# JerryX1110/Robust-Video-Object-Segmentation

Hardware: AMD Instinct MI355X
Metric: frames/sec, AOC-Net matching + calibration hot path (480p, 3 objects) (higher is better)
Workload: dtype f32; 1 GPU; cfg2: 121x213 stride-4 maps (480p), O=4 (3 objects + background), K=16 proxies, C=100, 60-frame clips, MEM_EVERY=5 (pool R=1..12), 20 Lloyd iterations, local windows 2..12, 10 IA gates + 4 conditioning blocks; sequences_per_gpu=2, proxy_mode=reference

## Files before the change

robust-video-object-segmentation_amd/csrc/labels_kmeans.hip:

```cpp
#include "aoc_common.h"
#include <stdlib.h>
#include <algorithm>

namespace {

constexpr int LP_BLOCK = 256;

__global__ __launch_bounds__(LP_BLOCK) void label_flags_kernel(const float *__restrict__ labels, int n, int n_obj,
                                                                uint32_t *__restrict__ right_bits,
                                                                uint32_t *__restrict__ wrong_bits,
                                                                int32_t *__restrict__ block_counts, int n_blocks) {
    __shared__ int32_t wave_cnt[LP_BLOCK / 64][AOC_MAX_OBJECTS + 1];
    const int row = blockIdx.x * LP_BLOCK + threadIdx.x;
    uint32_t right = 0, wrong = 0;
    if (row < n) {
        const float *l = labels + (size_t)row * n_obj;
        float sum = 0.0f;
        for (int o = 0; o < n_obj; ++o) {
            float v = l[o];
            sum += v;
            if (v > 0.9f) right |= 1u << o;
            if (v < 0.1f) wrong |= 1u << o;
        }
        if (sum > 0.9f) right |= AOC_ROW_KEPT_BIT;
// ... 285 lines not shown
        }
        float v[KU_G][NF];
#pragma unroll
        for (int u = 0; u < KU_G; ++u) {
            const float *base = pool + (size_t)r[u] * C;
#pragma unroll
            for (int f = 0; f < NF; ++f) {
                int t = lane + 64 * f;
                v[u][f] = (t < C) ? base[t] : 0.0f;
            }
        }
#pragma unroll
        for (int u = 0; u < KU_G; ++u) {
            const bool on = u < nmem;
#pragma unroll
            for (int f = 0; f < NF; ++f) acc[f] = acc[f] + (on ? v[u][f] : 0.0f);
        }
        qhead += nmem;
    };

    for (int base = 0; base < len; base += 64) {
        const int p = base + lane;
        const bool valid = p < len;
        const int lab = valid ? labels[beg + p] : -1;
        int row;
        if (MODE == 0) row = valid ? rows[beg + p] : 0;
        else row = valid ? rows[p] : 0;
        const bool mine = lab == j;
        const unsigned long long m = __ballot(mine);
        const int nm = __popcll(m);
        if (nm == 0) continue;
        if (mine) ring[(qtail + __popcll(m & lt)) & (KU_RING - 1)] = row;
        qtail += nm;
        cnt += nm;
        while (qtail - qhead >= KU_G) drain(KU_G);
    }
    while (qtail - qhead > 0) drain(min(KU_G, qtail - qhead));

    if (MODE == 0) {
        if (lane == 0) cluster_counts[s * kmax + j] = cnt;
        if (cnt == 0) return;
        const float fc = (float)cnt;
        float *dst = centroids + ((size_t)s * kmax + j) * C;
#pragma unroll
        for (int f = 0; f < NF; ++f) {
            int t = lane + 64 * f;
            float q = acc[f] / fc;
            if (t < C) { dst[t] = q; stage[t] = q; }
        }
        __syncthreads();
        if (lane == 0) cnorm[s * kmax + j] = sqnorm_seq(stage, C);
    } else {
        const float *csrc = centroids + ((size_t)s * kmax + j) * C;
        float *p0 = proxies + (((size_t)s * 2 + 0) * kmax + j) * C;
        float *p1 = proxies + (((size_t)s * 2 + 1) * kmax + j) * C;
        float n0 = 0.0f, n1 = 0.0f;
#pragma unroll
        for (int f = 0; f < NF; ++f) {
            int t = lane + 64 * f;
            if (t < C) {
                float c = csrc[t];
                p0[t] = c;
                n0 += c * c;
                float a = (cnt > 0) ? acc[f] / (float)cnt : 0.0f;
                p1[t] = a;
                n1 += a * a;
            }
        }
        n0 = aoc_wave_sum(n0);
        n1 = aoc_wave_sum(n1);
        if (lane == 0) {
            proxy_sqnorm[((size_t)s * 2 + 0) * kmax + j] = n0;
            proxy_sqnorm[((size_t)s * 2 + 1) * kmax + j] = (cnt > 0) ? n1 : INFINITY;
        }
    }
}

typedef uint32_t u32x4 __attribute__((ext_vector_type(4)));
typedef uint32_t u32x2 __attribute__((ext_vector_type(2)));
constexpr uint32_t KU_INVALID_OFF = 0xFFFFFF00u;

#ifdef AOC_KS_STATS
__device__ unsigned long long aoc_ks_stats[8];
#define KS_STAT(i, n) do { if (threadIdx.x == 0) atomicAdd(&aoc_ks_stats[i], (unsigned long long)(n)); } while (0)
#else
#define KS_STAT(i, n) do { } while (0)
#endif
#ifdef AOC_KS_STATS
#define KS_CLK() ((long long)__builtin_readcyclecounter())
#else
#define KS_CLK() 0ll
#endif
constexpr int KS_T = 8;

__device__ __forceinline__ int ks_wave_sum(int v) {
    v += __builtin_amdgcn_update_dpp(0, v, 0x111, 0xf, 0xf, true);
    v += __builtin_amdgcn_update_dpp(0, v, 0x112, 0xf, 0xf, true);
    v += __builtin_amdgcn_update_dpp(0, v, 0x114, 0xf, 0xf, true);
    v += __builtin_amdgcn_update_dpp(0, v, 0x118, 0xf, 0xf, true);
    return __builtin_amdgcn_readlane(v, 15) + __builtin_amdgcn_readlane(v, 31) + __builtin_amdgcn_readlane(v, 47) +
           __builtin_amdgcn_readlane(v, 63);
}

__device__ __forceinline__ void ks_fold_block(float x, float inv_u, int lane, int &accr, int &par, unsigned long long &badmask) {
    const float y = x * inv_u;
    const float rn = rintf(y);
    int r = (int)rn;
    badmask |= __ballot(!(__float_as_uint(y) < 0x4B800000u));
    const unsigned long long ties = __ballot(fabsf(rn - y) == 0.5f);
    if (ties) {
        const int fl = (int)floorf(y);
        if ((ties >> lane) & 1ull) r = fl;
        const unsigned long long odd = __ballot((r & 1) != 0);
        int base_par = par, from = 0;
        unsigned long long tm = ties;
        while (tm) {
            const int t = __builtin_ctzll(tm);
            tm &= tm - 1;
            const unsigned long long below_t = (t == 0) ? 0ull : (~0ull >> (64 - t));
            const unsigned long long below_from = (from == 0) ? 0ull : (~0ull >> (64 - from));
            const int pb = base_par ^ (__popcll(odd & below_t & ~below_from) & 1);
            const int bump = pb ^ (int)((odd >> t) & 1ull);
            if (lane == t) r += bump;
            base_par = 0;
            from = t + 1;
        }
        const unsigned long long rest = (from >= 64) ? 0ull : (~0ull << from);
        par = base_par ^ (__popcll(odd & rest) & 1);
    } else {
        par ^= __popcll(__ballot((r & 1) != 0)) & 1;
    }
    accr += r;
}

struct KsBinade {
    float u, inv_u;
    int n_in;
    bool ok;
};
__device__ __forceinline__ KsBinade ks_binade(float s) {
    KsBinade b;
    const uint32_t bits = __float_as_uint(s);
    const int e = (int)((bits >> 23) & 0xff) - 127;
    b.ok = (s > 0.0f) && e >= -100 && e <= 100;
    const int ee = b.ok ? e : 0;
    b.u = __uint_as_float((uint32_t)(ee - 23 + 127) << 23);
    b.inv_u = __uint_as_float((uint32_t)(23 - ee + 127) << 23);
    b.n_in = (int)(s * b.inv_u);
    return b;
}

__device__ __forceinline__ float ks_serial_block(float s, float x, int from = 0) {
    if (__ballot(x != 0.0f) == 0ull) return s;
    for (int kk = from; kk < 64; ++kk) s = s + __uint_as_float(__builtin_amdgcn_readlane(__float_as_uint(x), kk));
    return s;
}

__device__ __forceinline__ int ks_wave_scan(int v) {
    v += __builtin_amdgcn_update_dpp(0, v, 0x111, 0xf, 0xf, true);
    v += __builtin_amdgcn_update_dpp(0, v, 0x112, 0xf, 0xf, true);
    v += __builtin_amdgcn_update_dpp(0, v, 0x114, 0xf, 0xf, true);
    v += __builtin_amdgcn_update_dpp(0, v, 0x118, 0xf, 0xf, true);
    v += __builtin_amdgcn_update_dpp(0, v, 0x142, 0xa, 0xf, false);
    v += __builtin_amdgcn_update_dpp(0, v, 0x143, 0xc, 0xf, false);
    return v;
}

__device__ __forceinline__ float ks_block_exact(float s, float x, int lane) {
    int from = 0;
#pragma unroll 1
    for (int round = 0; round < 4; ++round) {
        const KsBinade bb = ks_binade(s);
        if (!bb.ok) break;
        int r = 0, pr = bb.n_in & 1;
        unsigned long long bd = 0ull;
        ks_fold_block((lane >= from) ? x : 0.0f, bb.inv_u, lane, r, pr, bd);
        if (bd != 0ull) break;
        const int pre = ks_wave_scan(r);
        const int total = __builtin_amdgcn_readlane(pre, 63);
        if ((long long)bb.n_in + total <= 0xFFFFFF) return (float)(bb.n_in + total) * bb.u;
        const unsigned long long over = __ballot((long long)bb.n_in + pre > 0xFFFFFF);
        const int mstar = __builtin_ctzll(over);
        const int before = (mstar == 0) ? 0 : __builtin_amdgcn_readlane(pre, mstar - 1);
        const float s_before = (float)(bb.n_in + before) * bb.u;
        s = s_before + __uint_as_float(__builtin_amdgcn_readlane(__float_as_uint(x), mstar));
        from = mstar + 1;
        if (from >= 64) return s;
    }
    return ks_serial_block(s, x, from);
}

template <int C4MAX>
__global__ __launch_bounds__(256) void km_assign_rank_kernel(const float *__restrict__ pool, int C, const int32_t *__restrict__ rows,
                                                              const int32_t *__restrict__ seg_off, const int32_t *__restrict__ seg_k,
                                                              const float *__restrict__ centroids, int kmax, int32_t *__restrict__ labels,
                                                              uint16_t *__restrict__ rank16, int32_t *__restrict__ hist, int nb_max,
                                                              float *__restrict__ rownorm, int first_iter) {
    extern __shared__ __attribute__((aligned(16))) float lds[];
    const int s = blockIdx.y;
    const int k = seg_k[s];
    if (k <= 0) return;
    const int beg = seg_off[s];
    const int len = seg_off[s + 1] - beg;
    if ((int)(blockIdx.x * 256) >= len) return;
    const int c4 = C >> 2;
    float *lc = lds;
    float *lcn = lds + (size_t)k * C;
    int32_t *wcnt = reinterpret_cast<int32_t *>(lcn + kmax);
    const float *csrc = centroids + (size_t)s * kmax * C;
    for (int i = threadIdx.x; i < k * C; i += 256) lc[i] = csrc[i];
    __syncthreads();
    if ((int)threadIdx.x < k) lcn[threadIdx.x] = sqnorm_seq(lc + (size_t)threadIdx.x * C, C);
    __syncthreads();
    const int p = blockIdx.x * 256 + threadIdx.x;
    const bool valid = p < len;
    int best = -1;
    if (valid) {
        const float4 *xr = reinterpret_cast<const float4 *>(pool + (size_t)rows[beg + p] * C);
        float4 x[C4MAX];
#pragma unroll
        for (int t = 0; t < C4MAX; ++t) x[t] = (t < c4) ? xr[t] : make_float4(0.f, 0.f, 0.f, 0.f);
        float xs;
        if (first_iter) {
            xs = 0.0f;
#pragma unroll
            for (int t = 0; t < C4MAX; ++t) {
                if (t < c4) {
                    float p0 = x[t].x * x[t].x; xs = xs + p0;
                    float p1 = x[t].y * x[t].y; xs = xs + p1;
                    float p2 = x[t].z * x[t].z; xs = xs + p2;
                    float p3 = x[t].w * x[t].w; xs = xs + p3;
                }
            }
            rownorm[beg + p] = xs;
        } else {
            xs = rownorm[beg + p];
        }
        float low = INFINITY;
        best = 0;
        for (int j = 0; j < k; ++j) {
            const float4 *cj = reinterpret_cast<const float4 *>(lc + (size_t)j * C);
            float acc = 0.0f;
#pragma unroll
            for (int t = 0; t < C4MAX; ++t) {
                if (t < c4) {
                    float4 c = cj[t];
                    acc = __builtin_fmaf(x[t].x, c.x, acc);
                    acc = __builtin_fmaf(x[t].y, c.y, acc);
                    acc = __builtin_fmaf(x[t].z, c.z, acc);
                    acc = __builtin_fmaf(x[t].w, c.w, acc);
                }
            }
            float m = -2.0f * acc;
            float dist = (m + xs) + lcn[j];
            if (dist < low) { low = dist; best = j; }
        }
        labels[beg + p] = best;
    }
    const int lane = aoc_lane(), wave = threadIdx.x >> 6;
    const unsigned long long lt = (lane == 0) ? 0ull : (~0ull >> (64 - lane));
    int rank = 0;
    for (int kk = 0; kk < k; ++kk) {
        const unsigned long long m = __ballot(best == kk);
        if (best == kk) rank = __popcll(m & lt);
        if (lane == 0) wcnt[wave * kmax + kk] = __popcll(m);
    }
    __syncthreads();
    if (valid) {
        int woff = 0;
        for (int w = 0; w < wave; ++w) woff += wcnt[w * kmax + best];
        rank16[beg + p] = (uint16_t)(woff + rank);
    }
    if ((int)threadIdx.x < k)
        hist[((size_t)s * nb_max + blockIdx.x) * kmax + threadIdx.x] =
            wcnt[threadIdx.x] + wcnt[kmax + threadIdx.x] + wcnt[2 * kmax + threadIdx.x] + wcnt[3 * kmax + threadIdx.x];
}

__global__ __launch_bounds__(256) void km_rownorm_kernel(const float *__restrict__ pool, int C, const int32_t *__restrict__ rows,
                                                          const int32_t *__restrict__ seg_off, int n_seg_limit, float *__restrict__ rownorm) {
    const int total = seg_off[n_seg_limit];
    const int i = blockIdx.x * 256 + threadIdx.x;
    if (i >= total) return;
    const float4 *xr = reinterpret_cast<const float4 *>(pool + (size_t)rows[i] * C);
    const int c4 = C >> 2;
    float xs = 0.0f;
    for (int t0 = 0; t0 < c4; t0 += 5) {
        float4 v[5];
#pragma unroll
        for (int u = 0; u < 5; ++u) v[u] = xr[min(t0 + u, c4 - 1)];
#pragma unroll
        for (int u = 0; u < 5; ++u) {
            if (t0 + u < c4) {
                float p0 = v[u].x * v[u].x; xs = xs + p0;
                float p1 = v[u].y * v[u].y; xs = xs + p1;
                float p2 = v[u].z * v[u].z; xs = xs + p2;
                float p3 = v[u].w * v[u].w; xs = xs + p3;
            }
        }
    }
    rownorm[i] = xs;
}

constexpr int KA_TPF4 = 1;
template <int TMAX, int KT>
__global__ __launch_bounds__(256, KT == 1 ? 3 : 2) void km_assign_mfma_kernel(const float *__restrict__ pool, int C, const int32_t *__restrict__ rows,
                                                              const int32_t *__restrict__ seg_off, const int32_t *__restrict__ seg_k, int n_seg,
                                                              const float *__restrict__ centroids, int kmax, int32_t *__restrict__ labels,
                                                              uint16_t *__restrict__ rank16, int32_t *__restrict__ hist, int nb_max,
                                                              const float *__restrict__ rownorm) {
    extern __shared__ __attribute__((aligned(16))) float lds[];
    constexpr int TP = (TMAX + 3) / 4 * 4;
    constexpr int RS = 4 * TP + 4;
    constexpr int NB4 = TP / 4;
    constexpr int PIECES = (16 * TMAX + 63) / 64;
    constexpr int c4 = TMAX;
    const int lane = aoc_lane(), wave = threadIdx.x >> 6;
    const int j = lane & 15, g = lane >> 4;

    float *cimg = lds;
    float *lcn = cimg + (size_t)KT * 16 * RS;
    float *wimg = lcn + KT * 16 + (size_t)wave * 16 * RS;
    int32_t *wcnt = reinterpret_cast<int32_t *>(lcn + KT * 16 + (size_t)4 * 16 * RS);

    if (TP > c4) {
        for (int idx = lane; idx < 16 * 4 * (TP - c4); idx += 64) {
            const int rr = idx / (4 * (TP - c4)), rem = idx - rr * 4 * (TP - c4);
            wimg[(size_t)rr * RS + (rem / (TP - c4)) * TP + c4 + rem % (TP - c4)] = 0.0f;
        }
        for (int idx = threadIdx.x; idx < KT * 16 * 4 * (TP - c4); idx += 256) {
            const int rr = idx / (4 * (TP - c4)), rem = idx - rr * 4 * (TP - c4);
            cimg[(size_t)rr * RS + (rem / (TP - c4)) * TP + c4 + rem % (TP - c4)] = 0.0f;
        }
    }

    constexpr int SEG_LDS = 128;
    __shared__ int32_t lseg_off[SEG_LDS + 1], lseg_nb[SEG_LDS];
    const bool seg_in_lds = n_seg <= SEG_LDS;
    if (seg_in_lds) {
        for (int i = threadIdx.x; i <= n_seg; i += 256) lseg_off[i] = seg_off[i];
        __syncthreads();
        for (int i = threadIdx.x; i < n_seg; i += 256) lseg_nb[i] = (seg_k[i] > 0) ? (lseg_off[i + 1] - lseg_off[i] + 255) / 256 : 0;
        __syncthreads();
    }

    float4 ca[KT][NB4];
    float cn[KT][4];
    int cur_seg = -1, k = 0, beg = 0, len = 0;
    for (int w = blockIdx.x;; w += gridDim.x) {
        int s = 0, bx = w;
        if (seg_in_lds) {
            for (; s < n_seg; ++s) {
                const int nbs = lseg_nb[s];
                if (bx < nbs) break;
                bx -= nbs;
            }
        } else {
            for (; s < n_seg; ++s) {
                const int ls = seg_off[s + 1] - seg_off[s];
                const int nbs = (seg_k[s] > 0) ? (ls + 255) / 256 : 0;
                if (bx < nbs) break;
                bx -= nbs;
            }
        }
        if (s >= n_seg) break;
        constexpr int TPF = KT >= 4 ? KA_TPF4 : 2;
        const int ibeg = seg_in_lds ? lseg_off[s] : seg_off[s], ilen = (seg_in_lds ? lseg_off[s + 1] : seg_off[s + 1]) - ibeg;
        const int wave_row0 = bx * 256 + wave * 64;
        float4 pv[TPF][PIECES];
        const int my_p = min(wave_row0 + lane, ilen - 1);
        const int my_id = rows[ibeg + max(my_p, 0)];
        const float my_xs = rownorm[ibeg + max(my_p, 0)];
        auto issue_tile = [&](int tile, float4 (&v)[PIECES]) {
#pragma unroll
            for (int i = 0; i < PIECES; ++i) {
                const int idx = min(i * 64 + lane, 16 * c4 - 1);
                const int rr = idx / c4, t = idx - rr * c4;
                const int id = __shfl(my_id, tile * 16 + rr);
                v[i] = reinterpret_cast<const float4 *>(pool + (size_t)id * C)[t];
            }
        };
        auto write_tile = [&](int tile, const float4 (&v)[PIECES]) {
#pragma unroll
            for (int i = 0; i < PIECES; ++i) {
                const int idx = i * 64 + lane;
                if (idx < 16 * c4) {
                    const int rr = idx / c4, t = idx - rr * c4;
                    const bool in = wave_row0 + tile * 16 + rr < ilen;
                    float *d = wimg + (size_t)rr * RS + t;
                    d[0] = in ? v[i].x : 0.f; d[TP] = in ? v[i].y : 0.f; d[2 * TP] = in ? v[i].z : 0.f; d[3 * TP] = in ? v[i].w : 0.f;
                }
            }
        };
#pragma unroll
        for (int t = 0; t < TPF; ++t) issue_tile(t, pv[t]);
        if (s != cur_seg) {
            cur_seg = s;
            k = seg_k[s];
            beg = seg_off[s];
            len = seg_off[s + 1] - beg;
            __syncthreads();
            const float *csrc = centroids + (size_t)s * kmax * C;
            for (int idx = threadIdx.x; idx < KT * 16 * c4; idx += 256) {
                const int cc = idx / c4, t = idx - cc * c4;
                const float4 v = (cc < k) ? reinterpret_cast<const float4 *>(csrc + (size_t)cc * C)[t] : make_float4(0.f, 0.f, 0.f, 0.f);
                float *d = cimg + (size_t)cc * RS + t;
                d[0] = v.x; d[TP] = v.y; d[2 * TP] = v.z; d[3 * TP] = v.w;
            }
            __syncthreads();
            if ((int)threadIdx.x < KT * 16) {
                float nrm = INFINITY;
                if ((int)threadIdx.x < k) {
                    const float *im = cimg + (size_t)threadIdx.x * RS;
                    nrm = 0.0f;
#pragma unroll
                    for (int t = 0; t < TMAX; ++t) {
                        if (t < c4) {
#pragma unroll
                            for (int kq = 0; kq < 4; ++kq) {
                                const float v = im[kq * TP + t];
                                const float prod = v * v;
                                nrm = nrm + prod;
                            }
                        }
                    }
                }
                lcn[threadIdx.x] = nrm;
            }
            __syncthreads();
#pragma unroll
            for (int kt = 0; kt < KT; ++kt) {
                const float *st = cimg + (size_t)(kt * 16 + j) * RS + g * TP;
#pragma unroll
                for (int u = 0; u < NB4; ++u) ca[kt][u] = *reinterpret_cast<const float4 *>(st + 4 * u);
#pragma unroll
                for (int r = 0; r < 4; ++r) cn[kt][r] = lcn[kt * 16 + g * 4 + r];
            }
        }

        int best = -1;
#pragma unroll
        for (int tile = 0; tile < 4; ++tile) {
            write_tile(tile, pv[tile % TPF]);
            if (tile + TPF < 4) issue_tile(tile + TPF, pv[tile % TPF]);
            const float *bs = wimg + (size_t)j * RS + g * TP;
            float4 xb[NB4];
#pragma unroll
            for (int u = 0; u < NB4; ++u) xb[u] = *reinterpret_cast<const float4 *>(bs + 4 * u);
            const int prow = wave_row0 + tile * 16 + j;
            const float xs_l = __shfl(my_xs, tile * 16 + j);
            const float xs = (prow < len) ? xs_l : 0.0f;
            float low = INFINITY;
            int arg = 0;
#pragma unroll
            for (int kt = 0; kt < KT; ++kt) {
                f32x4 acc = (f32x4){0.f, 0.f, 0.f, 0.f};
#pragma unroll
                for (int u = 0; u < NB4; ++u) {
                    const float aa[4] = {ca[kt][u].x, ca[kt][u].y, ca[kt][u].z, ca[kt][u].w};
                    const float bb[4] = {xb[u].x, xb[u].y, xb[u].z, xb[u].w};
#pragma unroll
                    for (int e = 0; e < 4; ++e)
                        if (4 * u + e < TMAX) acc = __builtin_amdgcn_mfma_f32_16x16x4f32(aa[e], bb[e], acc, 0, 0, 0);
                }
#pragma unroll
                for (int r = 0; r < 4; ++r) {
                    const float mm = -2.0f * acc[r];
                    const float dist = (mm + xs) + cn[kt][r];
                    if (dist < low) { low = dist; arg = kt * 16 + g * 4 + r; }
                }
            }
#pragma unroll
            for (int off = 16; off <= 32; off <<= 1) {
                const float d2 = __shfl_xor(low, off);
                const int a2 = __shfl_xor(arg, off);
                if (d2 < low || (d2 == low && a2 < arg)) { low = d2; arg = a2; }
            }
            const int mine = __shfl(arg, lane & 15);
            if ((lane >> 4) == tile) best = mine;
        }
        const int p = wave_row0 + lane;
        const bool valid = p < len;
        if (!valid) best = -1;
        if (valid) labels[beg + p] = best;
        const unsigned long long lt = (lane == 0) ? 0ull : (~0ull >> (64 - lane));
        int rank = 0;
        for (int kk = 0; kk < k; ++kk) {
            const unsigned long long mk = __ballot(best == kk);
            if (best == kk) rank = __popcll(mk & lt);
            if (lane == 0) wcnt[wave * kmax + kk] = __popcll(mk);
        }
        __syncthreads();
        if (valid) {
            int woff = 0;
            for (int ww = 0; ww < wave; ++ww) woff += wcnt[ww * kmax + best];
            rank16[beg + p] = (uint16_t)(woff + rank);
        }
        if ((int)threadIdx.x < k)
            hist[((size_t)s * nb_max + bx) * kmax + threadIdx.x] =
                wcnt[threadIdx.x] + wcnt[kmax + threadIdx.x] + wcnt[2 * kmax + threadIdx.x] + wcnt[3 * kmax + threadIdx.x];
        __syncthreads();
    }
}

template <int TMAX, int KT>
__global__ __launch_bounds__(256, KT == 1 ? 3 : 2) void km_assign_mfma_rep_kernel(const float *__restrict__ pool, int C, const int32_t *__restrict__ rows,
                                                                  const int32_t *__restrict__ seg_off, const int32_t *__restrict__ seg_k, int n_base,
                                                                  int n_rep, int n_grp, const float *__restrict__ centroids, int kmax,
                                                                  int32_t *__restrict__ labels, uint16_t *__restrict__ rank16,
                                                                  int32_t *__restrict__ hist, int nb_max, const float *__restrict__ rownorm) {
    extern __shared__ __attribute__((aligned(16))) float lds[];
    constexpr int TP = (TMAX + 3) / 4 * 4;
    constexpr int RS = 4 * TP + 4;
    constexpr int NB4 = TP / 4;
    constexpr int PIECES = (16 * TMAX + 63) / 64;
    constexpr int c4 = TMAX;
    constexpr int CB = KT * 16 * RS;
    constexpr int MAXG = 16;
    const int lane = aoc_lane(), wave = threadIdx.x >> 6;
    const int j = lane & 15, g = lane >> 4;

    float *cimg = lds;
    float *lcn = cimg + (size_t)n_grp * CB;
    float *wimg = lcn + (size_t)n_grp * KT * 16 + (size_t)wave * 16 * RS;
    int32_t *wcnt = reinterpret_cast<int32_t *>(lcn + (size_t)n_grp * KT * 16 + (size_t)4 * 16 * RS);
    uint8_t *lab = reinterpret_cast<uint8_t *>(wcnt + 4 * kmax);
    __shared__ int32_t lk[MAXG], lbeg[MAXG];

    if (TP > c4) {
        for (int idx = lane; idx < 16 * 4 * (TP - c4); idx += 64) {
            const int rr = idx / (4 * (TP - c4)), rem = idx - rr * 4 * (TP - c4);
            wimg[(size_t)rr * RS + (rem / (TP - c4)) * TP + c4 + rem % (TP - c4)] = 0.0f;
        }
        for (int idx = threadIdx.x; idx < n_grp * KT * 16 * 4 * (TP - c4); idx += 256) {
            const int rr = idx / (4 * (TP - c4)), rem = idx - rr * 4 * (TP - c4);
            cimg[(size_t)rr * RS + (rem / (TP - c4)) * TP + c4 + rem % (TP - c4)] = 0.0f;
        }
    }

    constexpr int SEG_LDS = 32;
    __shared__ int32_t lseg_off[SEG_LDS + 1], lseg_nb[SEG_LDS];
    const bool seg_in_lds = n_base <= SEG_LDS;
    auto seg_live = [&](int i) -> bool {
        bool any = false;
        for (int f = 0; f < n_rep; ++f) any |= seg_k[f * n_base + i] > 0;
        return any;
    };
    if (seg_in_lds) {
        for (int i = threadIdx.x; i <= n_base; i += 256) lseg_off[i] = seg_off[i];
        __syncthreads();
        for (int i = threadIdx.x; i < n_base; i += 256) lseg_nb[i] = seg_live(i) ? (lseg_off[i + 1] - lseg_off[i] + 255) / 256 : 0;
        __syncthreads();
    }
    int items_per_group = 0;
    for (int s = 0; s < n_base; ++s)
        items_per_group += seg_in_lds ? lseg_nb[s] : (seg_live(s) ? (seg_off[s + 1] - seg_off[s] + 255) / 256 : 0);
    const int n_groups = (n_rep + n_grp - 1) / n_grp;

    int cur_seg = -1, cur_grp = -1, ng = 0, len = 0;
    for (int w = blockIdx.x; items_per_group > 0; w += gridDim.x) {
        const int gi = w / items_per_group;
        if (gi >= n_groups) break;
        int s = 0, bx = w - gi * items_per_group;
        for (; s < n_base; ++s) {
            const int nbs = seg_in_lds ? lseg_nb[s] : (seg_live(s) ? (seg_off[s + 1] - seg_off[s] + 255) / 256 : 0);
            if (bx < nbs) break;
            bx -= nbs;
        }
        if (s >= n_base) break;
        constexpr int TPF = 2;
        const int ibeg = seg_in_lds ? lseg_off[s] : seg_off[s], ilen = (seg_in_lds ? lseg_off[s + 1] : seg_off[s + 1]) - ibeg;
        const int wave_row0 = bx * 256 + wave * 64;
        float4 pv[TPF][PIECES];
        const int my_p = min(wave_row0 + lane, ilen - 1);
        const int my_id = rows[ibeg + max(my_p, 0)];
        const float my_xs = rownorm[ibeg + max(my_p, 0)];
        auto issue_tile = [&](int tile, float4 (&v)[PIECES]) {
#pragma unroll
            for (int i = 0; i < PIECES; ++i) {
                const int idx = min(i * 64 + lane, 16 * c4 - 1);
                const int rr = idx / c4, t = idx - rr * c4;
                const int id = __shfl(my_id, tile * 16 + rr);
                v[i] = reinterpret_cast<const float4 *>(pool + (size_t)id * C)[t];
            }
        };
        auto write_tile = [&](int tile, const float4 (&v)[PIECES]) {
#pragma unroll
            for (int i = 0; i < PIECES; ++i) {
                const int idx = i * 64 + lane;
                if (idx < 16 * c4) {
                    const int rr = idx / c4, t = idx - rr * c4;
                    const bool in = wave_row0 + tile * 16 + rr < ilen;
                    float *d = wimg + (size_t)rr * RS + t;
                    d[0] = in ? v[i].x : 0.f; d[TP] = in ? v[i].y : 0.f; d[2 * TP] = in ? v[i].z : 0.f; d[3 * TP] = in ? v[i].w : 0.f;
                }
            }
        };
#pragma unroll
        for (int t = 0; t < TPF; ++t) issue_tile(t, pv[t]);
        if (s != cur_seg || gi != cur_grp) {
            cur_seg = s;
            cur_grp = gi;
            ng = min(n_grp, n_rep - gi * n_grp);
            len = ilen;
            __syncthreads();
            for (int r = 0; r < ng; ++r) {
                const int sr = (gi * n_grp + r) * n_base + s;
                const int kr = seg_k[sr];
                const float *csrc = centroids + (size_t)sr * kmax * C;
                float *ci = cimg + (size_t)r * CB;
                for (int idx = threadIdx.x; idx < KT * 16 * c4; idx += 256) {
                    const int cc = idx / c4, t = idx - cc * c4;
                    const float4 v = (cc < kr) ? reinterpret_cast<const float4 *>(csrc + (size_t)cc * C)[t] : make_float4(0.f, 0.f, 0.f, 0.f);
                    float *d = ci + (size_t)cc * RS + t;
                    d[0] = v.x; d[TP] = v.y; d[2 * TP] = v.z; d[3 * TP] = v.w;
                }
                if (threadIdx.x == 0) { lk[r] = kr; lbeg[r] = seg_off[sr]; }
            }
            __syncthreads();
            for (int idx = threadIdx.x; idx < ng * KT * 16; idx += 256) {
                const int r = idx / (KT * 16), cc = idx - r * (KT * 16);
                float nrm = INFINITY;
                if (cc < lk[r]) {
                    const float *im = cimg + (size_t)r * CB + (size_t)cc * RS;
                    nrm = 0.0f;
#pragma unroll
                    for (int t = 0; t < TMAX; ++t) {
#pragma unroll
                        for (int kq = 0; kq < 4; ++kq) {
                            const float v = im[kq * TP + t];
                            const float prod = v * v;
                            nrm = nrm + prod;
                        }
                    }
                }
                lcn[idx] = nrm;
            }
            __syncthreads();
        }

#pragma unroll
        for (int tile = 0; tile < 4; ++tile) {
            write_tile(tile, pv[tile % TPF]);
            if (tile + TPF < 4) issue_tile(tile + TPF, pv[tile % TPF]);
            const float *bs = wimg + (size_t)j * RS + g * TP;
            float4 xb[NB4];
#pragma unroll
            for (int u = 0; u < NB4; ++u) xb[u] = *reinterpret_cast<const float4 *>(bs + 4 * u);
            const int prow = wave_row0 + tile * 16 + j;
            const float xs_l = __shfl(my_xs, tile * 16 + j);
            const float xs = (prow < len) ? xs_l : 0.0f;
#pragma unroll 1
            for (int r = 0; r < ng; ++r) {
                float low = INFINITY;
                int arg = 0;
                const int ktr = (lk[r] + 15) >> 4;
#pragma unroll
                for (int kt = 0; kt < KT; ++kt) {
                    if (kt >= ktr) continue;
                    const float *st = cimg + (size_t)r * CB + (size_t)(kt * 16 + j) * RS + g * TP;
                    float4 ca[NB4];
#pragma unroll
                    for (int u = 0; u < NB4; ++u) ca[u] = *reinterpret_cast<const float4 *>(st + 4 * u);
                    const float4 cn4 = *reinterpret_cast<const float4 *>(lcn + (size_t)r * KT * 16 + kt * 16 + g * 4);
                    const float cn[4] = {cn4.x, cn4.y, cn4.z, cn4.w};
                    f32x4 acc = (f32x4){0.f, 0.f, 0.f, 0.f};
#pragma unroll
                    for (int u = 0; u < NB4; ++u) {
                        const float aa[4] = {ca[u].x, ca[u].y, ca[u].z, ca[u].w};
                        const float bb[4] = {xb[u].x, xb[u].y, xb[u].z, xb[u].w};
#pragma unroll
                        for (int e = 0; e < 4; ++e)
                            if (4 * u + e < TMAX) acc = __builtin_amdgcn_mfma_f32_16x16x4f32(aa[e], bb[e], acc, 0, 0, 0);
                    }
#pragma unroll
                    for (int q = 0; q < 4; ++q) {
                        const float mm = -2.0f * acc[q];
                        const float dist = (mm + xs) + cn[q];
                        if (dist < low) { low = dist; arg = kt * 16 + g * 4 + q; }
                    }
                }
#pragma unroll
                for (int off = 16; off <= 32; off <<= 1) {
                    const float d2 = __shfl_xor(low, off);
                    const int a2 = __shfl_xor(arg, off);
                    if (d2 < low || (d2 == low && a2 < arg)) { low = d2; arg = a2; }
                }
                const int mine = __shfl(arg, lane & 15);
                if ((lane >> 4) == tile) lab[r * 256 + threadIdx.x] = (uint8_t)mine;
            }
        }
        const int p = wave_row0 + lane;
        const bool valid = p < len;
        const unsigned long long lt = (lane == 0) ? 0ull : (~0ull >> (64 - lane));
        for (int r = 0; r < ng; ++r) {
            const int kr = lk[r], beg = lbeg[r];
            if (kr <= 0) continue;
            const int sr = (gi * n_grp + r) * n_base + s;
            const int best = valid ? (int)lab[r * 256 + threadIdx.x] : -1;
            if (valid) labels[beg + p] = best;
            int rank = 0;
            for (int kk = 0; kk < kr; ++kk) {
                const unsigned long long mk = __ballot(best == kk);
                if (best == kk) rank = __popcll(mk & lt);
                if (lane == 0) wcnt[wave * kmax + kk] = __popcll(mk);
            }
            __syncthreads();
            if (valid) {
                int woff = 0;
                for (int ww = 0; ww < wave; ++ww) woff += wcnt[ww * kmax + best];
                rank16[beg + p] = (uint16_t)(woff + rank);
            }
            if ((int)threadIdx.x < kr)
                hist[((size_t)sr * nb_max + bx) * kmax + threadIdx.x] =
                    wcnt[threadIdx.x] + wcnt[kmax + threadIdx.x] + wcnt[2 * kmax + threadIdx.x] + wcnt[3 * kmax + threadIdx.x];
            __syncthreads();
        }
    }
}

__global__ __launch_bounds__(256) void km_replicate_kernel(const int32_t *__restrict__ rows, const int32_t *__restrict__ seg_off,
                                                            const int32_t *__restrict__ seg_k, int n_seg, int n_rep, int64_t capacity,
                                                            int32_t *__restrict__ rows_out, int32_t *__restrict__ seg_off_out,
                                                            int32_t *__restrict__ seg_k_out) {
    const int64_t total = seg_off[n_seg];
    const int64_t i = (int64_t)blockIdx.x * blockDim.x + threadIdx.x;
    const int f = blockIdx.y;
    if (i < total && i < capacity) rows_out[f * total + i] = rows[i];
    if (i <= n_seg && (i < n_seg || f == n_rep - 1)) seg_off_out[f * n_seg + i] = (int32_t)(f * total + seg_off[i]);
    if (i < n_seg) seg_k_out[f * n_seg + i] = seg_k[i];
}

struct KmLevels {
    int32_t k[8];
    int32_t n;
};
__global__ __launch_bounds__(256) void km_replicate_levels_kernel(const int32_t *__restrict__ rows, const int32_t *__restrict__ seg_off,
                                                                   int n_seg, int n_rep, KmLevels klev, int64_t capacity,
                                                                   int32_t *__restrict__ rows_out, int32_t *__restrict__ seg_off_out,
                                                                   int32_t *__restrict__ seg_k_out) {
    const int64_t total = seg_off[n_seg];
    const int64_t i = (int64_t)blockIdx.x * blockDim.x + threadIdx.x;
    const int f = blockIdx.y;
    if (i < total && i < capacity && rows_out != rows) rows_out[f * total + i] = rows[i];
    if (i <= n_seg && (i < n_seg || f == n_rep - 1)) seg_off_out[f * n_seg + i] = (int32_t)(f * total + seg_off[i]);
    if (i < n_seg) {
        int k = klev.k[f % klev.n];
        for (int s = 0; s <= (int)i; ++s) k = min(k, seg_off[s + 1] - seg_off[s]);
        seg_k_out[f * n_seg + i] = k;
    }
}

__global__ __launch_bounds__(256) void km_rank_only_kernel(const int32_t *__restrict__ seg_off, const int32_t *__restrict__ seg_k,
                                                            const int32_t *__restrict__ labels, int kmax, uint16_t *__restrict__ rank16,
                                                            int32_t *__restrict__ hist, int nb_max) {
    __shared__ int32_t wcnt[4 * AOC_MAX_CLUSTERS];
    const int s = blockIdx.y;
    const int k = seg_k[s];
    if (k <= 0) return;
    const int beg = seg_off[s];
    const int len = seg_off[s + 1] - beg;
    if ((int)(blockIdx.x * 256) >= len) return;
    const int p = blockIdx.x * 256 + threadIdx.x;
    const bool valid = p < len;
    const int best = valid ? labels[beg + p] : -1;
    const int lane = aoc_lane(), wave = threadIdx.x >> 6;
    const unsigned long long lt = (lane == 0) ? 0ull : (~0ull >> (64 - lane));
    int rank = 0;
    for (int kk = 0; kk < k; ++kk) {
        const unsigned long long m = __ballot(best == kk);
        if (best == kk) rank = __popcll(m & lt);
        if (lane == 0) wcnt[wave * kmax + kk] = __popcll(m);
    }
    __syncthreads();
    if (valid) {
        int woff = 0;
        for (int w = 0; w < wave; ++w) woff += wcnt[w * kmax + best];
        rank16[beg + p] = (uint16_t)(woff + rank);
    }
    if ((int)threadIdx.x < k)
        hist[((size_t)s * nb_max + blockIdx.x) * kmax + threadIdx.x] =
            wcnt[threadIdx.x] + wcnt[kmax + threadIdx.x] + wcnt[2 * kmax + threadIdx.x] + wcnt[3 * kmax + threadIdx.x];
}

constexpr int KS_CHUNK = 64 * KS_T;
__host__ __device__ __forceinline__ int ks_seg_chunk_base(int seg_beg, int s, int kmax) { return seg_beg / KS_CHUNK + s * (kmax + 1); }
__host__ __device__ __forceinline__ int ks_seg_chunk_region(int len, int kmax) { return len / KS_CHUNK + kmax + 1; }

constexpr int KSS_BLOCKS = 8;
__global__ __launch_bounds__(256) void km_scan_scatter_kernel(const int32_t *__restrict__ rows, const int32_t *__restrict__ rows_local,
                                                               const int32_t *__restrict__ seg_off, const int32_t *__restrict__ seg_k, int n_seg,
                                                               const int32_t *__restrict__ labels, const uint16_t *__restrict__ rank16,
                                                               const int32_t *__restrict__ hist, int nb_max, int kmax, uint32_t row_bytes,
                                                               uint32_t *__restrict__ moff, int32_t *__restrict__ counts, int32_t *__restrict__ cbase,
                                                               int32_t *__restrict__ cchunk, int32_t *__restrict__ owner_cluster,
                                                               int32_t *__restrict__ owner_local, int nch_cap) {
    __shared__ int32_t part[2][256];
    __shared__ int32_t lpre[AOC_MAX_CLUSTERS], ltot[AOC_MAX_CLUSTERS], lbase[AOC_MAX_CLUSTERS];
    __shared__ int32_t loff[KSS_BLOCKS][AOC_MAX_CLUSTERS];
    __shared__ int32_t lchunk[AOC_MAX_CLUSTERS + 1];
    const int s = blockIdx.y;
    const int k = seg_k[s];
    const int beg = seg_off[s];
    const int len = seg_off[s + 1] - beg;
    const int b0 = blockIdx.x * KSS_BLOCKS;
    const bool first = blockIdx.x == 0;
    if (!first && (k <= 0 || b0 * 256 >= len)) return;
    const int nb = (k > 0) ? (len + 255) / 256 : 0;
    int kp = 1;
    while (kp < kmax) kp <<= 1;
    const int groups = 256 / kp;
    {
        const int kk = threadIdx.x & (kp - 1), g = threadIdx.x / kp;
        int pre = 0, tot = 0;
        if (kk < k) {
            const int32_t *hp = hist + (size_t)s * nb_max * kmax + kk;
            for (int bb = g; bb < nb; bb += 8 * groups) {
                int v[8];
#pragma unroll
                for (int u = 0; u < 8; ++u) v[u] = hp[(size_t)min(bb + u * groups, nb - 1) * kmax];
#pragma unroll
                for (int u = 0; u < 8; ++u) {
                    const int b = bb + u * groups;
                    const int w = (b < nb) ? v[u] : 0;
                    tot += w;
                    pre += (b < b0) ? w : 0;
                }
            }
        }
        part[0][threadIdx.x] = pre;
        part[1][threadIdx.x] = tot;
    }
    __syncthreads();
    if ((int)threadIdx.x < kmax) {
        int pre = 0, tot = 0;
        for (int g = 0; g < groups; ++g) {
            pre += part[0][g * kp + threadIdx.x];
            tot += part[1][g * kp + threadIdx.x];
        }
        lpre[threadIdx.x] = pre;
        ltot[threadIdx.x] = tot;
    }
    __syncthreads();
    if (threadIdx.x == 0) {
        const int cb = ks_seg_chunk_base(beg, s, kmax);
        int off = 0, ch = 0;
        for (int kk = 0; kk < kmax; ++kk) {
            lbase[kk] = off;
            lchunk[kk] = ch;
            if (first) {
                counts[s * kmax + kk] = ltot[kk];
                cbase[s * kmax + kk] = off;
                if (cchunk) cchunk[s * kmax + kk] = cb + ch;
            }
            off += ltot[kk];
            ch += (ltot[kk] + KS_CHUNK - 1) / KS_CHUNK;
        }
        lchunk[kmax] = ch;
    }
    if ((int)threadIdx.x < k) {
        int hv[KSS_BLOCKS];
#pragma unroll
        for (int i = 0; i < KSS_BLOCKS; ++i) hv[i] = hist[((size_t)s * nb_max + min(b0 + i, nb - 1)) * kmax + threadIdx.x];
        int run = lpre[threadIdx.x];
#pragma unroll
        for (int i = 0; i < KSS_BLOCKS; ++i) {
            loff[i][threadIdx.x] = run;
            run += (b0 + i < nb) ? hv[i] : 0;
        }
    }
    __syncthreads();
    if (first && owner_cluster) {
        const int cb = ks_seg_chunk_base(beg, s, kmax);
        const int region = ((s + 1 < n_seg) ? ks_seg_chunk_base(seg_off[s + 1], s + 1, kmax) : nch_cap) - cb;
        for (int i = threadIdx.x; i < region; i += 256) {
            int oc = -1, ol = 0;
            if (i < lchunk[kmax]) {
                int kk = 0;
                while (kk + 1 < kmax && lchunk[kk + 1] <= i) ++kk;
                oc = s * kmax + kk;
                ol = i - lchunk[kk];
            }
            owner_cluster[cb + i] = oc;
            owner_local[cb + i] = ol;
        }
    }
    if (k <= 0) return;
    int lab[KSS_BLOCKS], rk[KSS_BLOCKS], row[KSS_BLOCKS];
    const int32_t *rsrc = rows_local ? rows_local : rows + beg;
#pragma unroll
    for (int i = 0; i < KSS_BLOCKS; ++i) {
        const int p = min((b0 + i) * 256 + (int)threadIdx.x, len - 1);
        lab[i] = labels[beg + p];
        rk[i] = (int)rank16[beg + p];
        row[i] = rsrc[p];
    }
#pragma unroll
    for (int i = 0; i < KSS_BLOCKS; ++i) {
        const int p = (b0 + i) * 256 + threadIdx.x;
        if (p < len) moff[beg + lbase[lab[i]] + loff[i][lab[i]] + rk[i]] = (uint32_t)row[i] * row_bytes;
    }
}


__device__ __forceinline__ void kc_chunk_sum_body(int chunk, uint32_t *__restrict__ loffs, float4 *__restrict__ part,
                                                  const float *__restrict__ pool, int C, const int32_t *__restrict__ seg_off,
                                                  const int32_t *__restrict__ counts, const int32_t *__restrict__ cbase,
                                                  const uint32_t *__restrict__ moff, int kmax,
                                                  const int32_t *__restrict__ owner_cluster, const int32_t *__restrict__ owner_local,
                                                  float *__restrict__ csum, int start_chunk) {
    const int oc = owner_cluster[chunk];
    if (oc < 0) return;
    if (owner_local[chunk] < start_chunk) return;
    const int s = oc / kmax;
    const int cnt = counts[oc];
    const uint32_t *list = moff + seg_off[s] + cbase[oc];
    const int first = owner_local[chunk] * KS_CHUNK;
    const int members = min(KS_CHUNK, cnt - first);
    for (int i = threadIdx.x; i < KS_CHUNK; i += 256) loffs[i] = list[first + min(i, members - 1)];
    __syncthreads();
    const int c4 = C >> 2;
    const int rpp = 256 / c4;
    const int r0 = threadIdx.x / c4, piece = threadIdx.x - r0 * c4;
    const bool worker = r0 < rpp;
    float4 acc = make_float4(0.f, 0.f, 0.f, 0.f);
    if (worker) {
        const char *base = reinterpret_cast<const char *>(pool) + piece * 16;
        for (int m0 = r0; m0 < members; m0 += 8 * rpp) {
            float4 v[8];
#pragma unroll
            for (int u = 0; u < 8; ++u) v[u] = *reinterpret_cast<const float4 *>(base + loffs[min(m0 + u * rpp, KS_CHUNK - 1)]);
#pragma unroll
            for (int u = 0; u < 8; ++u) {
                if (m0 + u * rpp < members) { acc.x += v[u].x; acc.y += v[u].y; acc.z += v[u].z; acc.w += v[u].w; }
            }
        }
    }
    part[threadIdx.x] = acc;
    __syncthreads();
    if ((int)threadIdx.x < c4) {
        float4 t = part[threadIdx.x];
        for (int r = 1; r < rpp; ++r) {
            const float4 x = part[r * c4 + threadIdx.x];
            t.x += x.x; t.y += x.y; t.z += x.z; t.w += x.w;
        }
        *reinterpret_cast<float4 *>(csum + (size_t)chunk * C + 4 * threadIdx.x) = t;
    }
}

constexpr int KC_UNSAFE = -128;
__device__ __forceinline__ int kc_predict_binade(float pre, float end) {
    int e = KC_UNSAFE;
    if (pre > 1e-30f && end < 1e30f && end >= pre) {
        const int e_lo = (int)((__float_as_uint(pre * 0.9995f) >> 23) & 0xff) - 127;
        const int e_hi = (int)((__float_as_uint(end * 1.0005f) >> 23) & 0xff) - 127;
        if (e_lo == e_hi && e_lo >= -100 && e_lo <= 100) e = e_lo;
    }
    return e;
}
constexpr int KP_CROSS = 4;
struct KsPred {
    int8_t *e0;
    uint16_t *cidx;
    int8_t *ce;
};
__device__ __forceinline__ int kp_predict(const KsPred &p, size_t idx, int c) {
    int e = p.e0[idx];
#pragma unroll
    for (int i = 0; i < KP_CROSS; ++i) {
        const int ci = p.cidx[idx * KP_CROSS + i];
        if (e == KC_UNSAFE || ci == 0xFFFF || c < ci) break;
        e = (c == ci) ? KC_UNSAFE : (int)p.ce[idx * KP_CROSS + i];
    }
    return e;
}
__global__ __launch_bounds__(128) void km_chunk_predict_kernel(const int32_t *__restrict__ seg_k, const int32_t *__restrict__ counts,
                                                                const int32_t *__restrict__ cchunk, const float *__restrict__ csum, int kmax,
                                                                int C, int8_t *__restrict__ cexp, int start_chunk,
                                                                const float *__restrict__ head_state) {
    const int s = blockIdx.y, j = blockIdx.x;
    if (j >= seg_k[s]) return;
    const int oc = s * kmax + j;
    const int nch = (counts[oc] + KS_CHUNK - 1) / KS_CHUNK;
    if (nch <= start_chunk) return;
    const int base = cchunk[oc];
    for (int f = threadIdx.x; f < C; f += blockDim.x) {
        float pre = (start_chunk > 0) ? head_state[(size_t)oc * C + f] : 0.0f;
        for (int c0 = start_chunk; c0 < nch; c0 += 8) {
          float cs[8];
#pragma unroll
          for (int u = 0; u < 8; ++u) cs[u] = (c0 + u < nch) ? csum[(size_t)(base + c0 + u) * C + f] : 0.0f;
#pragma unroll
          for (int u = 0; u < 8; ++u) {
            const int c = c0 + u;
            if (c >= nch) break;
            const float end = pre + cs[u];
            cexp[(size_t)(base + c) * C + f] = (int8_t)kc_predict_binade(pre, end);
            pre = end;
          }
        }
    }
}

struct KcFold {
    int acc;
    int par0, par1;
    int bump0, bump1;
    int bad;
};
__device__ __forceinline__ void kc_fold_block2(float x, float inv_u, KcFold &k) {
    const float y = x * inv_u;
    const float rn = rintf(y);
    int r = (int)rn;
    k.bad |= (__ballot(!(__float_as_uint(y) < 0x4B800000u)) != 0ull) ? 1 : 0;
    const unsigned long long ties = __ballot(fabsf(rn - y) == 0.5f);
    if (ties) {
        const int lane = aoc_lane();
        if ((ties >> lane) & 1ull) r = (int)floorf(y);
        const unsigned long long odd = __ballot((r & 1) != 0);
        int pp[2] = {k.par0, k.par1}, bb[2] = {0, 0};
// ... 1161 lines not shown
```

Measured before the change: 445.3 frames/s.

## Use contiguous work runs with prefetched next item in k-means assign kernels

Replaces the grid-stride item loop with a contiguous per-block run of work items, and prefetches the next item's segment lookup, row ids and norms while the current item computes. It uses 32-bit byte offsets for pool loads, swaps the xor shuffles in the argmin reduction for permlane16/32 swap builtins, and makes the wave index uniform. In the grouped kernel, the per-group histogram and rank pass now uses one barrier pair instead of two barriers per group, by staging counts and ranks in the per-wave LDS scratch. This adds register pressure and assumes pool offsets fit in 32 bits and that pool rows are 16*TMAX bytes apart (C == 4*TMAX).

```diff
diff --git a/robust-video-object-segmentation_amd/csrc/labels_kmeans.hip b/robust-video-object-segmentation_amd/csrc/labels_kmeans.hip
--- a/robust-video-object-segmentation_amd/csrc/labels_kmeans.hip
+++ b/robust-video-object-segmentation_amd/csrc/labels_kmeans.hip
@@ -611,6 +611,20 @@
 }
 
 constexpr int KA_TPF4 = 1;
+__device__ __forceinline__ void km_item_run(int n_items, int &w, int &w_end) {
+    const int grid = (int)gridDim.x, b = (int)blockIdx.x;
+    const int base = n_items / grid, rem = n_items - base * grid;
+    w = b * base + min(b, rem);
+    w_end = w + base + (b < rem ? 1 : 0);
+}
+__device__ __forceinline__ int km_lane_xor(int x, int off, int lane) {
+    if (off == 16) {
+        const auto r = __builtin_amdgcn_permlane16_swap((unsigned)x, (unsigned)x, false, false);
+        return (int)((lane & 16) ? r[0] : r[1]);
+    }
+    const auto r = __builtin_amdgcn_permlane32_swap((unsigned)x, (unsigned)x, false, false);
+    return (int)((lane & 32) ? r[0] : r[1]);
+}
 template <int TMAX, int KT>
 __global__ __launch_bounds__(256, KT == 1 ? 3 : 2) void km_assign_mfma_kernel(const float *__restrict__ pool, int C, const int32_t *__restrict__ rows,
                                                               const int32_t *__restrict__ seg_off, const int32_t *__restrict__ seg_k, int n_seg,
@@ -623,7 +637,7 @@
     constexpr int NB4 = TP / 4;
     constexpr int PIECES = (16 * TMAX + 63) / 64;
     constexpr int c4 = TMAX;
-    const int lane = aoc_lane(), wave = threadIdx.x >> 6;
+    const int lane = aoc_lane(), wave = __builtin_amdgcn_readfirstlane(threadIdx.x >> 6);
     const int j = lane & 15, g = lane >> 4;
 
     float *cimg = lds;
@@ -655,39 +669,49 @@
     float4 ca[KT][NB4];
     float cn[KT][4];
     int cur_seg = -1, k = 0, beg = 0, len = 0;
-    for (int w = blockIdx.x;; w += gridDim.x) {
-        int s = 0, bx = w;
-        if (seg_in_lds) {
-            for (; s < n_seg; ++s) {
-                const int nbs = lseg_nb[s];
-                if (bx < nbs) break;
-                bx -= nbs;
-            }
-        } else {
-            for (; s < n_seg; ++s) {
-                const int ls = seg_off[s + 1] - seg_off[s];
-                const int nbs = (seg_k[s] > 0) ? (ls + 255) / 256 : 0;
-                if (bx < nbs) break;
-                bx -= nbs;
-            }
-        }
-        if (s >= n_seg) break;
-        constexpr int TPF = KT >= 4 ? KA_TPF4 : 2;
-        const int ibeg = seg_in_lds ? lseg_off[s] : seg_off[s], ilen = (seg_in_lds ? lseg_off[s + 1] : seg_off[s + 1]) - ibeg;
+    auto seg_blocks = [&](int i) -> int {
+        return seg_in_lds ? lseg_nb[i] : ((seg_k[i] > 0) ? (seg_off[i + 1] - seg_off[i] + 255) / 256 : 0);
+    };
+    int n_items = 0;
+    for (int i = 0; i < n_seg; ++i) n_items += seg_blocks(i);
+    int w, w_end;
+    km_item_run(n_items, w, w_end);
+    constexpr int TPF = KT >= 4 ? KA_TPF4 : 2;
+    auto open_item = [&](int ww, int &s_, int &bx_, int &ilen_, int &id_, float &xs_) {
+        bx_ = ww;
+        for (s_ = 0; s_ < n_seg - 1; ++s_) {
+            const int nbs = seg_blocks(s_);
+            if (bx_ < nbs) break;
+            bx_ -= nbs;
+        }
+        const int ibeg = seg_in_lds ? lseg_off[s_] : seg_off[s_];
+        ilen_ = (seg_in_lds ? lseg_off[s_ + 1] : seg_off[s_ + 1]) - ibeg;
+        const int p = max(min(bx_ * 256 + wave * 64 + lane, ilen_ - 1), 0);
+        id_ = rows[ibeg + p];
+        xs_ = rownorm[ibeg + p];
+    };
+    auto issue_tile = [&](int ids, int tile, float4 (&v)[PIECES]) {
+#pragma unroll
+        for (int i = 0; i < PIECES; ++i) {
+            const int idx = min(i * 64 + lane, 16 * c4 - 1);
+            const int rr = idx / c4, t = idx - rr * c4;
+            const int id = __shfl(ids, tile * 16 + rr);
+            const uint32_t off = (uint32_t)id * (uint32_t)(16 * c4) + (uint32_t)(16 * t);
+            v[i] = *reinterpret_cast<const float4 *>(reinterpret_cast<const char *>(pool) + off);
+        }
+    };
+    int s = 0, bx = 0, ilen = 0, my_id = 0;
+    float my_xs = 0.0f;
+    if (w < w_end) open_item(w, s, bx, ilen, my_id, my_xs);
+    for (; w < w_end; ++w) {
+        float4 pv[TPF][PIECES];
+#pragma unroll
+        for (int t = 0; t < TPF; ++t) issue_tile(my_id, t, pv[t]);
+        const bool more = w + 1 < w_end;
+        int ns = s, nbx = bx, nilen = ilen, nid = my_id;
+        float nxs = my_xs;
+        if (more) open_item(w + 1, ns, nbx, nilen, nid, nxs);
         const int wave_row0 = bx * 256 + wave * 64;
-        float4 pv[TPF][PIECES];
-        const int my_p = min(wave_row0 + lane, ilen - 1);
-        const int my_id = rows[ibeg + max(my_p, 0)];
-        const float my_xs = rownorm[ibeg + max(my_p, 0)];
-        auto issue_tile = [&](int tile, float4 (&v)[PIECES]) {
-#pragma unroll
-            for (int i = 0; i < PIECES; ++i) {
-                const int idx = min(i * 64 + lane, 16 * c4 - 1);
-                const int rr = idx / c4, t = idx - rr * c4;
-                const int id = __shfl(my_id, tile * 16 + rr);
-                v[i] = reinterpret_cast<const float4 *>(pool + (size_t)id * C)[t];
-            }
-        };
         auto write_tile = [&](int tile, const float4 (&v)[PIECES]) {
 #pragma unroll
             for (int i = 0; i < PIECES; ++i) {
@@ -700,8 +724,6 @@
                 }
             }
         };
-#pragma unroll
-        for (int t = 0; t < TPF; ++t) issue_tile(t, pv[t]);
         if (s != cur_seg) {
             cur_seg = s;
             k = seg_k[s];
@@ -750,7 +772,7 @@
 #pragma unroll
         for (int tile = 0; tile < 4; ++tile) {
             write_tile(tile, pv[tile % TPF]);
-            if (tile + TPF < 4) issue_tile(tile + TPF, pv[tile % TPF]);
+            if (tile + TPF < 4) issue_tile(my_id, tile + TPF, pv[tile % TPF]);
             const float *bs = wimg + (size_t)j * RS + g * TP;
             float4 xb[NB4];
 #pragma unroll
@@ -780,8 +802,8 @@
             }
 #pragma unroll
             for (int off = 16; off <= 32; off <<= 1) {
-                const float d2 = __shfl_xor(low, off);
-                const int a2 = __shfl_xor(arg, off);
+                const float d2 = __int_as_float(km_lane_xor(__float_as_int(low), off, lane));
+                const int a2 = km_lane_xor(arg, off, lane);
                 if (d2 < low || (d2 == low && a2 < arg)) { low = d2; arg = a2; }
             }
             const int mine = __shfl(arg, lane & 15);
@@ -808,6 +830,7 @@
             hist[((size_t)s * nb_max + bx) * kmax + threadIdx.x] =
                 wcnt[threadIdx.x] + wcnt[kmax + threadIdx.x] + wcnt[2 * kmax + threadIdx.x] + wcnt[3 * kmax + threadIdx.x];
         __syncthreads();
+        s = ns; bx = nbx; ilen = nilen; my_id = nid; my_xs = nxs;
     }
 }
 
@@ -825,7 +848,7 @@
     constexpr int c4 = TMAX;
     constexpr int CB = KT * 16 * RS;
     constexpr int MAXG = 16;
-    const int lane = aoc_lane(), wave = threadIdx.x >> 6;
+    const int lane = aoc_lane(), wave = __builtin_amdgcn_readfirstlane(threadIdx.x >> 6);
     const int j = lane & 15, g = lane >> 4;
 
     float *cimg = lds;
@@ -865,33 +888,47 @@
         items_per_group += seg_in_lds ? lseg_nb[s] : (seg_live(s) ? (seg_off[s + 1] - seg_off[s] + 255) / 256 : 0);
     const int n_groups = (n_rep + n_grp - 1) / n_grp;
 
+    const int n_items = items_per_group * n_groups;
+    int w, w_end;
+    km_item_run(n_items, w, w_end);
+    constexpr int TPF = 2;
+    auto open_item = [&](int ww, int &gi_, int &s_, int &bx_, int &ilen_, int &id_, float &xs_) {
+        gi_ = ww / items_per_group;
+        bx_ = ww - gi_ * items_per_group;
+        for (s_ = 0; s_ < n_base - 1; ++s_) {
+            const int nbs = seg_in_lds ? lseg_nb[s_] : (seg_live(s_) ? (seg_off[s_ + 1] - seg_off[s_] + 255) / 256 : 0);
+            if (bx_ < nbs) break;
+            bx_ -= nbs;
+        }
+        const int ibeg = seg_in_lds ? lseg_off[s_] : seg_off[s_];
+        ilen_ = (seg_in_lds ? lseg_off[s_ + 1] : seg_off[s_ + 1]) - ibeg;
+        const int p = max(min(bx_ * 256 + wave * 64 + lane, ilen_ - 1), 0);
+        id_ = rows[ibeg + p];
+        xs_ = rownorm[ibeg + p];
+    };
+    auto issue_tile = [&](int ids, int tile, float4 (&v)[PIECES]) {
+#pragma unroll
+        for (int i = 0; i < PIECES; ++i) {
+            const int idx = min(i * 64 + lane, 16 * c4 - 1);
+            const int rr = idx / c4, t = idx - rr * c4;
+            const int id = __shfl(ids, tile * 16 + rr);
+            const uint32_t off = (uint32_t)id * (uint32_t)(16 * c4) + (uint32_t)(16 * t);
+            v[i] = *reinterpret_cast<const float4 *>(reinterpret_cast<const char *>(pool) + off);
+        }
+    };
+    int gi = 0, s = 0, bx = 0, ilen = 0, my_id = 0;
+    float my_xs = 0.0f;
+    if (w < w_end) open_item(w, gi, s, bx, ilen, my_id, my_xs);
     int cur_seg = -1, cur_grp = -1, ng = 0, len = 0;
-    for (int w = blockIdx.x; items_per_group > 0; w += gridDim.x) {
-        const int gi = w / items_per_group;
-        if (gi >= n_groups) break;
-        int s = 0, bx = w - gi * items_per_group;
-        for (; s < n_base; ++s) {
-            const int nbs = seg_in_lds ? lseg_nb[s] : (seg_live(s) ? (seg_off[s + 1] - seg_off[s] + 255) / 256 : 0);
-            if (bx < nbs) break;
-            bx -= nbs;
-        }
-        if (s >= n_base) break;
-        constexpr int TPF = 2;
-        const int ibeg = seg_in_lds ? lseg_off[s] : seg_off[s], ilen = (seg_in_lds ? lseg_off[s + 1] : seg_off[s + 1]) - ibeg;
+    for (; w < w_end; ++w) {
+        float4 pv[TPF][PIECES];
+#pragma unroll
+        for (int t = 0; t < TPF; ++t) issue_tile(my_id, t, pv[t]);
+        const bool more = w + 1 < w_end;
+        int ngi = gi, ns = s, nbx = bx, nilen = ilen, nid = my_id;
+        float nxs = my_xs;
+        if (more) open_item(w + 1, ngi, ns, nbx, nilen, nid, nxs);
         const int wave_row0 = bx * 256 + wave * 64;
-        float4 pv[TPF][PIECES];
-        const int my_p = min(wave_row0 + lane, ilen - 1);
-        const int my_id = rows[ibeg + max(my_p, 0)];
-        const float my_xs = rownorm[ibeg + max(my_p, 0)];
-        auto issue_tile = [&](int tile, float4 (&v)[PIECES]) {
-#pragma unroll
-            for (int i = 0; i < PIECES; ++i) {
-                const int idx = min(i * 64 + lane, 16 * c4 - 1);
-                const int rr = idx / c4, t = idx - rr * c4;
-                const int id = __shfl(my_id, tile * 16 + rr);
-                v[i] = reinterpret_cast<const float4 *>(pool + (size_t)id * C)[t];
-            }
-        };
         auto write_tile = [&](int tile, const float4 (&v)[PIECES]) {
 #pragma unroll
             for (int i = 0; i < PIECES; ++i) {
@@ -904,8 +941,6 @@
                 }
             }
         };
-#pragma unroll
-        for (int t = 0; t < TPF; ++t) issue_tile(t, pv[t]);
         if (s != cur_seg || gi != cur_grp) {
             cur_seg = s;
             cur_grp = gi;
@@ -950,7 +985,7 @@
 #pragma unroll
         for (int tile = 0; tile < 4; ++tile) {
             write_tile(tile, pv[tile % TPF]);
-            if (tile + TPF < 4) issue_tile(tile + TPF, pv[tile % TPF]);
+            if (tile + TPF < 4) issue_tile(my_id, tile + TPF, pv[tile % TPF]);
             const float *bs = wimg + (size_t)j * RS + g * TP;
             float4 xb[NB4];
 #pragma unroll
@@ -990,8 +1025,8 @@
                 }
 #pragma unroll
                 for (int off = 16; off <= 32; off <<= 1) {
-                    const float d2 = __shfl_xor(low, off);
-                    const int a2 = __shfl_xor(arg, off);
+                    const float d2 = __int_as_float(km_lane_xor(__float_as_int(low), off, lane));
+                    const int a2 = km_lane_xor(arg, off, lane);
                     if (d2 < low || (d2 == low && a2 < arg)) { low = d2; arg = a2; }
                 }
                 const int mine = __shfl(arg, lane & 15);
@@ -1001,29 +1036,42 @@
         const int p = wave_row0 + lane;
         const bool valid = p < len;
         const unsigned long long lt = (lane == 0) ? 0ull : (~0ull >> (64 - lane));
+        constexpr int WS = 16 * RS;
+        int32_t *mycnt = reinterpret_cast<int32_t *>(wimg);
+        uint8_t *myrank = reinterpret_cast<uint8_t *>(mycnt + ng * kmax);
         for (int r = 0; r < ng; ++r) {
-            const int kr = lk[r], beg = lbeg[r];
+            const int kr = lk[r];
             if (kr <= 0) continue;
-            const int sr = (gi * n_grp + r) * n_base + s;
             const int best = valid ? (int)lab[r * 256 + threadIdx.x] : -1;
-            if (valid) labels[beg + p] = best;
-            int rank = 0;
+            if (valid) labels[lbeg[r] + p] = best;
+            int rank = 0, cnt = 0;
             for (int kk = 0; kk < kr; ++kk) {
                 const unsigned long long mk = __ballot(best == kk);
                 if (best == kk) rank = __popcll(mk & lt);
-                if (lane == 0) wcnt[wave * kmax + kk] = __popcll(mk);
-            }
-            __syncthreads();
+                if (lane == kk) cnt = __popcll(mk);
+            }
+            if (lane < kr) mycnt[r * kmax + lane] = cnt;
+            myrank[r * 64 + lane] = (uint8_t)rank;
+        }
+        __syncthreads();
+        const int32_t *cnt0 = mycnt - (size_t)wave * WS;
+        for (int r = 0; r < ng; ++r) {
+            const int kr = lk[r];
+            if (kr <= 0) continue;
+            const int sr = (gi * n_grp + r) * n_base + s;
             if (valid) {
+                const int best = (int)lab[r * 256 + threadIdx.x];
                 int woff = 0;
-                for (int ww = 0; ww < wave; ++ww) woff += wcnt[ww * kmax + best];
-                rank16[beg + p] = (uint16_t)(woff + rank);
-            }
-            if ((int)threadIdx.x < kr)
-                hist[((size_t)sr * nb_max + bx) * kmax + threadIdx.x] =
-                    wcnt[threadIdx.x] + wcnt[kmax + threadIdx.x] + wcnt[2 * kmax + threadIdx.x] + wcnt[3 * kmax + threadIdx.x];
-            __syncthreads();
-        }
+                for (int ww = 0; ww < wave; ++ww) woff += cnt0[ww * WS + r * kmax + best];
+                rank16[lbeg[r] + p] = (uint16_t)(woff + (int)myrank[r * 64 + lane]);
+            }
+            if ((int)threadIdx.x < kr) {
+                const int32_t *c = cnt0 + r * kmax + threadIdx.x;
+                hist[((size_t)sr * nb_max + bx) * kmax + threadIdx.x] = c[0] + c[WS] + c[2 * WS] + c[3 * WS];
+            }
+        }
+        __syncthreads();
+        gi = ngi; s = ns; bx = nbx; ilen = nilen; my_id = nid; my_xs = nxs;
     }
 }
 
```

Measured after the change: 447.7 frames/s (median of 6 runs). Within noise of the previous version (+0.6%).
